# congkaishen/MotionPlanning

Hardware: AMD Instinct MI355X
Metric: MPPI rollouts/s (K×H dyn+cost steps/s) at K=8192,H=50; 1/2/4/8 GPU (higher is better)
Workload: dtype f64

## Files before the change

motionplanning_amd/csrc/mppi.hip:

```cpp
#include "mppi_device.hpp"
#include "runtime.hpp"

#include <hip/hip_ext.h>

#include <algorithm>
#include <cstdlib>
#include <type_traits>
#include <vector>

using namespace mpk;

namespace {

constexpr int NT = 256;
constexpr int RPB = NT / 2;
#ifndef MPPI_PRIO
#define MPPI_PRIO 3
#endif
constexpr size_t kMaxLds = 146 * 1024;
constexpr size_t kCoLds = 70 * 1024;

__device__ __forceinline__ double block_reduce_min(double v, double* sh) {
  for (int o = 32; o >= 1; o >>= 1) v = nanmin(v, __shfl_xor(v, o));
  const int w = threadIdx.x >> 6;
// ... 39 lines not shown
  int* rc_out;
  int* fc_out;
  int nb;
  int pstride;
  int lds_unom, lds_obs, lds_grid;
  int lds_cq;
  int lds_ctrl, lds_part;
  unsigned long long* stamps;
  int inline_noise;
  double* fin;
  int fin_stride;
  const int* live;
};

#ifndef MPPI_NT_CTRL
#define MPPI_NT_CTRL 0
#endif

struct FinRec {
  int u, unom, x0, goal, obs, grid, ran, stride;
  __host__ __device__ FinRec(int H, int n_obs, int gbytes) {
    u = 0;
    unom = 2 * H;
    x0 = 4 * H;
    goal = x0 + 7;
    obs = goal + 2;
    grid = obs + 3 * n_obs;
    ran = grid + (gbytes + 7) / 8;
    stride = (ran + 2) & ~1;
  }
};

#define MP_STAMP(i)                                                                  \
  do {                                                                               \
    if (A.stamps && threadIdx.x == 0) {                                              \
      A.stamps[blockIdx.x * 32 + (i)] = __builtin_amdgcn_s_memrealtime();            \
      if ((i) == 0) {                                                                \
        unsigned xcc;                                                                \
        asm volatile("s_getreg_b32 %0, hwreg(HW_REG_XCC_ID)" : "=s"(xcc));           \
        A.stamps[blockIdx.x * 32 + 30] = xcc;                                        \
      }                                                                              \
    }                                                                                \
  } while (0)
#define MP_STAMP_WAVE()                                                              \
  do {                                                                               \
    if (A.stamps && (threadIdx.x & 63) == 0) {                                       \
      unsigned hwid;                                                                 \
      asm volatile("s_getreg_b32 %0, hwreg(HW_REG_HW_ID)" : "=s"(hwid));             \
      A.stamps[blockIdx.x * 32 + 8 + (threadIdx.x >> 6)] = __builtin_amdgcn_s_memrealtime(); \
      A.stamps[blockIdx.x * 32 + 20 + (threadIdx.x >> 6)] = hwid;                    \
    }                                                                                \
  } while (0)

__global__ __launch_bounds__(256) void noise_prep_kernel(MppiDev P, int S, const double* ext, double* zh) {
  const long long i = (long long)blockIdx.x * blockDim.x + threadIdx.x;
  const long long n = (long long)S * P.H * P.K;
  if (i >= n) return;
  const int k = (int)(i % P.K);
  const long long t = i / P.K;
  const int h = (int)(t % P.H), s = (int)(t / P.H);
  double z[2];
  if (P.noise_mode == 0) {
    const double2 e = *reinterpret_cast<const double2*>(ext + (((size_t)s * P.K + k) * P.H + h) * 2);
    z[0] = e.x;
    z[1] = e.y;
  } else {
    philox_normal2(P, (unsigned)s, (unsigned)k, (unsigned)h, z);
  }
  reinterpret_cast<double2*>(zh)[i] = make_double2(z[0], z[1]);
}

template <class T>
__device__ __forceinline__ void st_ag(T* p, T v) {
  __hip_atomic_store(p, v, __ATOMIC_RELAXED, __HIP_MEMORY_SCOPE_AGENT);
}
template <class T>
__device__ __forceinline__ T ld_ag(const T* p) {
  return __hip_atomic_load(const_cast<T*>(p), __ATOMIC_RELAXED, __HIP_MEMORY_SCOPE_AGENT);
}
#ifndef MPPI_COHERENT_PARTS
#define MPPI_COHERENT_PARTS 0
#endif

template <int BT, int LPR, bool INL>
__global__ __launch_bounds__(BT) void mppi_plan_kernel(MppiDev P, PlanArgs A) {
  constexpr int NT = BT, RPB = BT / LPR, NQ = BT / 128;
  constexpr bool WPART = LPR == 2;
  __shared__ double sh_red[NT / 64];
  __shared__ double sh_e[RPB];
  __shared__ double sh_q[WPART ? NT / 64 : NQ][128];
  __shared__ int sh_last, sh_m, sh_bstar, sh_fc;
  __shared__ double sh_eta;
  __shared__ double atab[kTabDoubles];
  extern __shared__ double dyn[];
  const int H = P.H, H2 = 2 * H, K = P.K;
  const int s = blockIdx.x / A.nb, b = blockIdx.x % A.nb;
  const int tid = threadIdx.x, pair = LPR == 2 ? tid >> 1 : tid, side = LPR == 2 ? tid & 1 : 0;
  const int k = b * RPB + pair;
  const bool active = k < K;
  const int kk = active ? k : K - 1;
  if (A.live && A.live[s] == 0) {
    if (A.fin && b == 0 && tid == 0) A.fin[(size_t)s * A.fin_stride + FinRec(H, P.n_obs, P.gnx * P.gny).ran] = 0.0;
    return;
  }
  MP_STAMP(0);
  __builtin_amdgcn_s_setprio(3);

  const double* X0 = A.X0 + 7 * s;
  const double* goal = A.goal + 2 * s;
  const double* noise = A.noise ? A.noise + (size_t)K * H2 * s : nullptr;
  double* unom = dyn + A.lds_unom;
  double* obs = A.obs ? dyn + A.lds_obs : nullptr;
  double* ush = A.lds_ctrl >= 0 ? dyn + A.lds_ctrl : nullptr;
  const int ustr = H2 + 1;
  const unsigned char* grid = nullptr;
  {
    const double* gu = A.unom + (size_t)H2 * s;
    rollout_tab_fill(atab, P, tid, NT);
    for (int i = tid; i < H2; i += NT) unom[i] = gu[i];
    if (P.ctrl_cost)
      for (int i = tid; i < H; i += NT) ctrl_cost_row(P, gu[2 * i], gu[2 * i + 1], dyn + A.lds_cq + 2 * i);
    if (A.obs) {
      const double* go = A.obs + (size_t)3 * P.n_obs * s;
      for (int i = tid; i < 3 * P.n_obs; i += NT) obs[i] = go[i];
    }
    if (A.grid) {
      const int gb = P.gnx * P.gny;
      const unsigned char* gg = A.grid + (size_t)gb * s;
      if (A.lds_grid >= 0) {
        unsigned char* lg = reinterpret_cast<unsigned char*>(dyn + A.lds_grid);
        for (int i = tid; i < gb; i += NT) lg[i] = gg[i];
        grid = lg;
      } else {
        grid = gg;
      }
    }
    __syncthreads();
  }
  double* ctrl_g = A.ctrl_all ? A.ctrl_all + ((size_t)s * H * K + kk) * 2 + side : nullptr;

#if MPPI_PRIO == 3
  __shared__ int sh_simd[NT / 64];
  __shared__ volatile int sh_prog[NT / 64];
  const int wv = __builtin_amdgcn_readfirstlane(tid >> 6);
  int sib = -1;
  {
    unsigned hw;
    asm volatile("s_getreg_b32 %0, hwreg(HW_REG_HW_ID)" : "=s"(hw));
    if ((tid & 63) == 0) {
      sh_simd[wv] = (int)((hw >> 4) & 3u);
      sh_prog[wv] = 0;
    }
    __syncthreads();
    const int me = sh_simd[wv];
    for (int w = 0; w < NT / 64; w++)
      if (w != wv && sh_simd[w] == me) sib = w;
    sib = __builtin_amdgcn_readfirstlane(sib);
  }
  int sib_j = 0;
#endif
  int feas;
  double c;
  {
    const double2* zrow = noise ? reinterpret_cast<const double2*>(noise) + kk : nullptr;
    double2 zc = zrow ? zrow[0] : make_double2(0.0, 0.0), zn = zc;
    auto ctrl = [&](int j, double* u) {
      double2 zj;
      if (INL && LPR == 1) {
        double zz[2];
        philox_normal2(P, (unsigned)s, (unsigned)kk, (unsigned)j, zz);
        zj = make_double2(zz[0], zz[1]);
      } else if (INL) {
        if ((j & 1) == 0) {
          double zz[2];
          philox_normal2(P, (unsigned)s, (unsigned)kk, (unsigned)(j + side), zz);
          const double o0 = pair_swap(zz[0]), o1 = pair_swap(zz[1]);
          zj = side ? make_double2(o0, o1) : make_double2(zz[0], zz[1]);
          zn = side ? make_double2(zz[0], zz[1]) : make_double2(o0, o1);
        } else {
          zj = zn;
        }
      } else {
        zj = zc;
        if (j + 1 < H) zc = zrow[(size_t)(j + 1) * K];
      }
      const double z[2] = {zj.x, zj.y};
      sample_ctrl(P, z, unom + 2 * j, u);
#if MPPI_PRIO == 0
      if ((4 * j) % H < 4 && j > 0) {
        const int q = (4 * j) / H;
        if (q == 1) __builtin_amdgcn_s_setprio(2);
        else if (q == 2) __builtin_amdgcn_s_setprio(1);
        else if (q == 3) __builtin_amdgcn_s_setprio(0);
      }
#elif MPPI_PRIO == 3
      if (sib >= 0) {
        const int o = __builtin_amdgcn_readfirstlane(sib_j);
        if (j > o) __builtin_amdgcn_s_setprio(0);
        else if (j < o) __builtin_amdgcn_s_setprio(2);
        else __builtin_amdgcn_s_setprio(1);
        sh_prog[wv] = j;
        sib_j = sh_prog[sib];
      } else if ((4 * j) % H < 4 && j > 0) {
        const int q = (4 * j) / H;
        if (q == 1) __builtin_amdgcn_s_setprio(2);
        else if (q == 2) __builtin_amdgcn_s_setprio(1);
        else if (q == 3) __builtin_amdgcn_s_setprio(0);
      }
#else
      if (j > 0) {
        const int t1 = MPPI_PRIO == 1 ? H / 2 : H - 12, t2 = MPPI_PRIO == 1 ? 3 * H / 4 : H - 6,
                  t3 = MPPI_PRIO == 1 ? 7 * H / 8 : H - 3;
        if (j == t1) __builtin_amdgcn_s_setprio(2);
        else if (j == t2) __builtin_amdgcn_s_setprio(1);
        else if (j == t3) __builtin_amdgcn_s_setprio(0);
      }
#endif
    };
    auto store = [&](int j, const double* u) {
      if (LPR == 2) {
        if (ush) ush[pair * ustr + 2 * j + side] = u[side];
        if (ctrl_g) {
#if MPPI_NT_CTRL
          __builtin_nontemporal_store(u[side], ctrl_g + (size_t)j * K * 2);
#else
          ctrl_g[(size_t)j * K * 2] = u[side];
#endif
        }
      } else {
        if (ush) {
          ush[pair * ustr + 2 * j] = u[0];
          ush[pair * ustr + 2 * j + 1] = u[1];
        }
        if (ctrl_g) *reinterpret_cast<double2*>(ctrl_g + (size_t)j * K * 2) = make_double2(u[0], u[1]);
      }
    };
    const TrajOut traj{A.coll_traj ? A.coll_traj + (size_t)s * (H + 1) * 7 * K + kk : nullptr, 7LL * K, (long long)K};
    c = rollout_pair<LPR>(P, X0, goal, obs, grid, unom, side, ctrl, store, traj, &feas, atab, dyn + A.lds_cq);
  }
  MP_STAMP(1);
  MP_STAMP_WAVE();
  if (active && side == 0) {
    st_ag(A.cost_all + (size_t)s * K + k, c);
    st_ag(A.feas_all + (size_t)s * K + k, (unsigned char)feas);
    if (c != c) atomicOr(A.flags, 1);
  }
  const int wid = tid >> 6, lane = tid & 63;
  const bool wp = WPART && H2 <= 128;
  const int nr = wp ? max(0, min(32, K - b * RPB - 32 * wid)) : 0;
  constexpr bool PREF = BT == 512;
  double v0[32], v1[32];
  if (PREF && wp && !ush) {
    asm volatile("s_waitcnt vmcnt(0)" ::: "memory");
    const double* cb = A.ctrl_all + (((size_t)s * H + (lane >> 1)) * K + (size_t)b * RPB + 32 * wid) * 2 + (lane & 1);
    const size_t up = (size_t)64 * K;
#pragma unroll
    for (int r = 0; r < 32; r++) v0[r] = (r < nr && lane < H2) ? cb[2 * r] : 0.0;
    if (H2 > 64) {
#pragma unroll
      for (int r = 0; r < 32; r++) v1[r] = (r < nr && lane + 64 < H2) ? cb[up + 2 * r] : 0.0;
    }
  }
  const double cm = active ? c : __builtin_inf();
  const double rho_b = block_reduce_min(cm, sh_red);
  const double e = active ? mpj_exp(P.nil * (c - rho_b)) : 0.0;
  if (side == 0) sh_e[pair] = e;
  const double eta_b = block_reduce_sum(side == 0 ? e : 0.0, sh_red);
  const double fc_b = block_reduce_sum((side == 0 && active && feas) ? 1.0 : 0.0, sh_red);
  __syncthreads();
  double* part = A.part + ((size_t)s * A.nb + b) * A.pstride;
  if (wp) {
    const double* ew = sh_e + 32 * wid;
    double a0 = 0.0, a1 = 0.0;
    if (ush) {
      const double* uw = ush + (size_t)(32 * wid) * ustr + lane;
      for (int r = 0; r < nr; r++) {
        const double er = ew[r];
        if (lane < H2) a0 = a0 + er * uw[r * ustr];
        if (lane + 64 < H2) a1 = a1 + er * uw[r * ustr + 64];
      }
    } else if (PREF) {
#pragma unroll
      for (int r = 0; r < 32; r++) {
        if (r < nr) {
          const double er = ew[r];
          a0 = a0 + er * v0[r];
          if (H2 > 64) a1 = a1 + er * v1[r];
        }
      }
    } else {
      const double* cb = A.ctrl_all + (((size_t)s * H + (lane >> 1)) * K + (size_t)b * RPB + 32 * wid) * 2 + (lane & 1);
      const size_t up = (size_t)64 * K;
      for (int r = 0; r < nr; r++) {
        const double er = ew[r];
        if (lane < H2) a0 = a0 + er * cb[2 * r];
        if (lane + 64 < H2) a1 = a1 + er * cb[up + 2 * r];
      }
    }
    sh_q[wid][lane] = a0;
    sh_q[wid][lane + 64] = a1;
    __syncthreads();
    if (tid < H2) {
      double v = sh_q[0][tid];
#pragma unroll
      for (int w = 1; w < NT / 64; w++) v = v + sh_q[w][tid];
      st_ag(part + 4 + tid, v);
    }
  } else {
    const int t = tid % 128, q = tid / 128;
    const int r0 = q * (RPB / NQ), r1 = r0 + RPB / NQ;
    for (int t0 = 0; t0 < H2; t0 += 128) {
      const int tt = t0 + t;
      double acc = 0.0;
      if (tt < H2) {
        if (ush) {
          for (int r = r0; r < r1; r++) acc = acc + sh_e[r] * ush[r * ustr + tt];
        } else {
          const double* cb = A.ctrl_all + (((size_t)s * H + (tt >> 1)) * K + (size_t)b * RPB) * 2 + (tt & 1);
          const int rmax = min(r1, K - b * RPB);
#pragma unroll 16
          for (int r = r0; r < rmax; r++) acc = acc + sh_e[r] * cb[(size_t)r * 2];
// ... 328 lines not shown
      for (int k = 0; k < 7; k++) states[7 * vv + k] = x[k];
      if (last >= max_steps) live[vv] = 0;
    }
  }
}

__host__ __device__ inline int shard_rec(int H) { return 2 * H + 7 * (H + 1) + 4; }

__global__ __launch_bounds__(256) void shard_pack_kernel(int S, int H, const double* U, const double* traj,
                                                         const double* cost, const int* feas, const int* rc,
                                                         const int* fc, double* out) {
  const int D = shard_rec(H), nu = 2 * H, nt = 7 * (H + 1);
  const long long i = (long long)blockIdx.x * 256 + threadIdx.x;
  if (i >= (long long)S * D) return;
  const int s = (int)(i / D), j = (int)(i % D);
  double v;
  if (j < nu) v = U[(size_t)s * nu + j];
  else if (j < nu + nt) v = traj[(size_t)s * nt + (j - nu)];
  else {
    const int q = j - nu - nt;
    v = q == 0 ? cost[s] : q == 1 ? (double)feas[s] : q == 2 ? (double)rc[s] : (double)fc[s];
  }
  out[i] = v;
}

static void inv2(const double* A, double* Ai) {
  const double a = A[0], b = A[1], c = A[2], d = A[3];
  if (b == 0.0 && c == 0.0) {
    Ai[0] = 1.0 / a; Ai[1] = 0.0; Ai[2] = 0.0; Ai[3] = 1.0 / d;
    return;
  }
  const bool swap = __builtin_fabs(c) > __builtin_fabs(a);
  const double p11 = swap ? c : a, p12 = swap ? d : b, q11 = swap ? a : c, q12 = swap ? b : d;
  const double l = q11 / p11, u22 = q12 - l * p12;
  const double iu11 = 1.0 / p11, iu22 = 1.0 / u22, iu12 = -(p12 * iu11) * iu22;
  const double m11 = iu11 - iu12 * l, m12 = iu12, m21 = -iu22 * l, m22 = iu22;
  if (swap) { Ai[0] = m12; Ai[1] = m11; Ai[2] = m22; Ai[3] = m21; }
  else { Ai[0] = m11; Ai[1] = m12; Ai[2] = m21; Ai[3] = m22; }
}

static int make_dev_params(mp_ctx* ctx, const mp_mppi_params* p, int K, MppiDev* D) {
  MP_CHECK(ctx, p != nullptr, "params is NULL");
  MP_CHECK(ctx, K >= 1, "SamplingNumber K (%d) must be >= 1", K);
  MP_CHECK(ctx, p->H >= 1 && p->H <= 4096, "horizon N (%d) must be in [1, 4096]", p->H);
  MP_CHECK(ctx, p->n_obs >= 0, "n_obs (%d) must be >= 0", p->n_obs);
  MP_CHECK(ctx, p->dt > 0.0, "dt (%g) must be > 0", p->dt);
  MP_CHECK(ctx, p->grid_nx >= 0 && p->grid_ny >= 0, "grid dims must be >= 0");
  MP_CHECK(ctx, p->noise_mode == MP_NOISE_EXTERNAL || p->noise_mode == MP_NOISE_PHILOX, "bad noise_mode %d",
           p->noise_mode);
  MP_CHECK(ctx, p->calls_in_flight >= 0 && p->calls_in_flight <= 64, "calls_in_flight (%d) must be in [0, 64]",
           p->calls_in_flight);
  D->in_flight = p->calls_in_flight > 1 ? p->calls_in_flight : 1;
  D->K = K;
  D->H = p->H;
  D->FC = p->feasibility_count;
  D->n_obs = p->n_obs;
  D->dt = p->dt;
  D->lambda = p->lambda;
  D->nil = (-1.0) / p->lambda;
  const double* S = p->sigma;
  MP_CHECK(ctx, S[0] > 0.0, "Σ must be positive definite");
  const double l11 = __builtin_sqrt(S[0]);
  const double l21 = S[2] / l11;
  const double r22 = S[3] - l21 * l21;
  MP_CHECK(ctx, r22 > 0.0, "Σ must be positive definite");
  D->L[0] = l11; D->L[1] = 0.0; D->L[2] = l21; D->L[3] = __builtin_sqrt(r22);
  inv2(S, D->Si);
  for (int i = 0; i < 7; i++) { D->XL[i] = p->XL[i]; D->XU[i] = p->XU[i]; }
  for (int i = 0; i < 2; i++) { D->CL[i] = p->CL[i]; D->CU[i] = p->CU[i]; }
  D->slack = p->slack_penalty;
  D->obs_pen = p->obs_penalty;
  D->gnx = p->grid_nx;
  D->gny = p->grid_ny;
  D->gx0 = p->grid_x0; D->gy0 = p->grid_y0; D->gdx = p->grid_dx; D->gdy = p->grid_dy;
  D->noise_mode = p->noise_mode;
  D->ctrl_cost = p->ctrl_cost;
  D->seed = p->seed;
  D->offset = p->offset;
  D->scene_base = p->scene_base;
  return MP_OK;
}

using PlanFn = void (*)(MppiDev, PlanArgs);
static PlanFn plan_kernel_for(int BT, int LPR, bool inl) {
#define MP_PLAN_CASE(bt, lpr) \
  if (BT == bt && LPR == lpr) return inl ? mppi_plan_kernel<bt, lpr, true> : mppi_plan_kernel<bt, lpr, false>;
  MP_PLAN_CASE(128, 1)
  MP_PLAN_CASE(128, 2)
  MP_PLAN_CASE(256, 1)
  MP_PLAN_CASE(256, 2)
  MP_PLAN_CASE(512, 1)
  MP_PLAN_CASE(512, 2)
#undef MP_PLAN_CASE
  return nullptr;
}

static int plan_launch(mp_ctx* ctx, const MppiDev& D, int S, const double* X0, const double* goal,
                       const double* U_nom, const double* obstacles, const uint8_t* grid, const double* noise,
                       double* U_out, double* traj_out, double* cost_out, int32_t* feasible_out,
                       int32_t* rc_out, int32_t* fc_out, double* coll_traj, double* coll_ctrl,
                       double* coll_cost, uint8_t* coll_feas, int final_stream, const int* live = nullptr) {
  const int K = D.K, H = D.H;
  const char* lpr_s = getenv("MPGPU_LPR");
  const int lpr_env = lpr_s ? atoi(lpr_s) : 0;
  const int LPR = lpr_env == 1 || lpr_env == 2 ? lpr_env : ((size_t)S * K * D.in_flight >= 131072 ? 1 : 2);
  const int BT = LPR == 1 ? ((size_t)S * ((K + 511) / 512) >= 256 ? 512 : 256)
                          : ((size_t)S * ((K + 255) / 256) >= 256 ? 512 : 256);
  const int RPBh = BT / LPR;
  const int nb = (K + RPBh - 1) / RPBh;
  const int pstride = 4 + 2 * H;
  PlanArgs A;
  A.live = live;
  A.X0 = X0; A.goal = goal; A.unom = U_nom; A.obs = D.n_obs > 0 ? obstacles : nullptr;
  A.grid = D.gnx > 0 ? grid : nullptr;
  A.inline_noise = D.noise_mode == MP_NOISE_PHILOX;
  A.noise = nullptr;
  if (!A.inline_noise) {
    double* zh = (double*)mp_ws(ctx, WS_NOISE, sizeof(double) * (size_t)S * K * H * 2);
    if (!zh) return MP_ERR_NOMEM;
    const long long n = (long long)S * K * H;
    hipLaunchKernelGGL(noise_prep_kernel, dim3((unsigned)((n + 255) / 256)), dim3(256), 0, ctx->stream, D, S, noise,
                       zh);
    MP_HIP(ctx, hipGetLastError());
    A.noise = zh;
  }
  A.cost_all = coll_cost ? coll_cost : (double*)mp_ws(ctx, WS_MPPI_COST, sizeof(double) * (size_t)S * K);
  A.feas_all = coll_feas ? coll_feas : (unsigned char*)mp_ws(ctx, WS_MPPI_FEAS, (size_t)S * K);
  A.part = (double*)mp_ws(ctx, WS_MPPI_PART, sizeof(double) * (size_t)S * nb * pstride);
  if (!A.cost_all || !A.feas_all || !A.part) return MP_ERR_NOMEM;
  A.coll_traj = coll_traj;
  int st = mp_ticket_reserve(ctx, S);
  if (st) return st;
  A.tickets = ctx->tickets;
  A.flags = ctx->flags;
  A.U_out = U_out; A.traj_out = traj_out; A.cost_out = cost_out; A.feas_out = feasible_out;
  A.rc_out = rc_out; A.fc_out = fc_out;
  A.nb = nb;
  A.pstride = pstride;
  int off = 2 * H + nb;
  A.lds_unom = off;
  off += 2 * H;
  A.lds_cq = off;
  off += 2 * H;
  A.lds_obs = off;
  off += 3 * D.n_obs;
  const size_t gbytes = (size_t)D.gnx * D.gny;
  A.lds_grid = -1;
  if (D.gnx > 0 && (size_t)off * 8 + gbytes <= 48 * 1024) {
    A.lds_grid = off;
    off += (int)((gbytes + 7) / 8);
  }
  const int ctrl_words = RPBh * (2 * H + 1), part_words = nb * pstride;
  A.lds_ctrl = A.lds_part = -1;
  const bool many = (size_t)S * nb > 256;
  const size_t budget = many ? kCoLds : kMaxLds;
  if ((size_t)(off + (ctrl_words > part_words ? ctrl_words : part_words)) * 8 <= budget) {
    A.lds_ctrl = A.lds_part = off;
    off += ctrl_words > part_words ? ctrl_words : part_words;
  } else if ((size_t)(off + part_words) * 8 <= budget) {
    A.lds_part = off;
    off += part_words;
  }
  A.ctrl_all = coll_ctrl;
  if (A.lds_ctrl < 0 && !A.ctrl_all) {
    A.ctrl_all = (double*)mp_ws(ctx, WS_IO14, sizeof(double) * (size_t)S * K * 2 * H);
    if (!A.ctrl_all) return MP_ERR_NOMEM;
  }
  const size_t shmem = sizeof(double) * (size_t)off;
  MP_CHECK(ctx, shmem <= kMaxLds, "K/H/obstacles too large for one scene (dynamic LDS %zu B)", shmem);
  if (!ctx->mppi_lds_attr) {
    MP_HIP(ctx, hipSetDevice(ctx->device));
    for (int bt : {128, 256, 512})
      for (int lpr : {1, 2})
        for (bool inl : {false, true})
          MP_HIP(ctx, hipFuncSetAttribute((const void*)plan_kernel_for(bt, lpr, inl),
                                          hipFuncAttributeMaxDynamicSharedMemorySize, (int)kMaxLds));
    ctx->mppi_lds_attr = true;
  }
  A.fin = nullptr;
  A.fin_stride = 0;
  int par = 0;
  if (final_stream) {
    int st2 = mp_side_init(ctx);
    if (st2) return st2;
    par = ctx->fin_par;
    ctx->fin_par = (par + 1) % MP_FIN_RING;
    const FinRec R(H, D.n_obs, D.gnx * D.gny);
    A.fin_stride = R.stride;
    for (int q = 0; q < MP_FIN_RING; q++)
      if (!mp_ws(ctx, WS_FIN0 + q, sizeof(double) * (size_t)S * R.stride)) return MP_ERR_NOMEM;
    A.fin = (double*)mp_ws(ctx, WS_FIN0 + par, sizeof(double) * (size_t)S * R.stride);
    MP_HIP(ctx, hipEventSynchronize(ctx->ev_fin[par]));
  }
  A.stamps = nullptr;
  static const bool stamps_on = getenv("MPGPU_STAMPS") != nullptr;
  if (stamps_on) {
    A.stamps = (unsigned long long*)mp_ws(ctx, WS_HA2, sizeof(unsigned long long) * 32 * S * nb);
    MP_HIP(ctx, hipMemsetAsync(A.stamps, 0, sizeof(unsigned long long) * 32 * S * nb, ctx->stream));
  }
  hipEvent_t t_start, t_stop;
  mp_time_pair(ctx, &t_start, &t_stop);
  const dim3 grd(S * nb);
  {
    MppiDev Dl = D;
    void* args[] = {(void*)&Dl, (void*)&A};
    MP_HIP(ctx, hipExtLaunchKernel((const void*)plan_kernel_for(BT, LPR, A.inline_noise != 0), grd, dim3(BT), args,
                                   shmem, ctx->stream, t_start, t_stop, 0));
  }
  MP_HIP(ctx, hipGetLastError());
  if (final_stream) {
    const FinRec R(H, D.n_obs, D.gnx * D.gny);
    const int grid_lds = (size_t)R.stride * 8 <= 64 * 1024;
    const size_t fsh = sizeof(double) * (size_t)(grid_lds ? R.stride : R.grid);
    MP_CHECK(ctx, fsh <= kMaxLds, "final rollout snapshot too large for LDS (%zu B)", fsh);
    if (!ctx->fin_lds_attr) {
      MP_HIP(ctx, hipSetDevice(ctx->device));
      MP_HIP(ctx, hipFuncSetAttribute((const void*)final_rollout_kernel, hipFuncAttributeMaxDynamicSharedMemorySize,
                                      (int)kMaxLds));
      ctx->fin_lds_attr = true;
    }
    hipEvent_t plan_done = t_stop;
    if (!plan_done) {
      plan_done = ctx->ev_plan[par];
      MP_HIP(ctx, hipEventRecord(plan_done, ctx->stream));
    }
    MP_HIP(ctx, hipStreamWaitEvent(ctx->side, plan_done, 0));
    hipLaunchKernelGGL(final_rollout_kernel, dim3(S), dim3(64), fsh, ctx->side, D, A.fin, A.fin_stride, grid_lds,
                       traj_out, cost_out, feasible_out, ctx->flags);
    MP_HIP(ctx, hipGetLastError());
    MP_HIP(ctx, hipEventRecord(ctx->ev_fin[par], ctx->side));
  }
  if (stamps_on) {
    std::vector<unsigned long long> h(32 * S * nb);
    MP_HIP(ctx, hipMemcpyAsync(h.data(), A.stamps, h.size() * 8, hipMemcpyDeviceToHost, ctx->stream));
    MP_HIP(ctx, hipStreamSynchronize(ctx->stream));
    unsigned long long t0 = ~0ull, end = 0;
    double d01 = 0, d12 = 0, d23 = 0;
    int last = -1;
    for (int b = 0; b < S * nb; b++) {
      const unsigned long long* q = &h[32 * b];
      t0 = q[0] < t0 ? q[0] : t0;
      d01 += (q[1] - q[0]) / 100.0; d12 += (q[2] - q[1]) / 100.0; d23 += (q[3] - q[2]) / 100.0;
      if (q[5]) last = b;
      end = q[5] > end ? q[5] : end;
      end = q[3] > end ? q[3] : end;
    }
    fprintf(stderr, "[stamps us] blocks=%d mean rollout %.2f partial %.2f ticket %.2f", S * nb, d01 / (S * nb),
            d12 / (S * nb), d23 / (S * nb));
    {
      std::vector<double> st, en;
      for (int b = 0; b < S * nb; b++) {
        st.push_back((h[32 * b] - t0) / 100.0);
        en.push_back((h[32 * b + 1] - t0) / 100.0);
      }
      std::sort(st.begin(), st.end());
      std::sort(en.begin(), en.end());
      const int n = S * nb;
      fprintf(stderr, " | start p0/50/90/100 %.1f %.1f %.1f %.1f | p1-end p0/50/90/100 %.1f %.1f %.1f %.1f", st[0],
              st[n / 2], st[n * 9 / 10], st[n - 1], en[0], en[n / 2], en[n * 9 / 10], en[n - 1]);
      std::vector<double> we;
      int hist[9] = {0};
      for (int b = 0; b < n; b++) {
        int cnt[4] = {0, 0, 0, 0}, mx = 0;
        for (int w = 0; w < 8; w++) {
          const unsigned long long tw = h[32 * b + 8 + w];
          if (!tw) continue;
          we.push_back((tw - t0) / 100.0);
          const int simd = (int)((h[32 * b + 20 + w] >> 4) & 3);
          mx = std::max(mx, ++cnt[simd]);
        }
        hist[mx]++;
      }
      std::sort(we.begin(), we.end());
      const int m = (int)we.size();
      fprintf(stderr, " | wave-end p0/50/90/100 %.1f %.1f %.1f %.1f | blocks by max waves/SIMD 1:%d 2:%d 3:%d 4:%d",
              we[0], we[m / 2], we[m * 9 / 10], we[m - 1], hist[1], hist[2], hist[3], hist[4]);
    }
    {
      double sum[16] = {0}, mx[16] = {0};
      int cnt[16] = {0}, nbk[16] = {0};
      for (int b = 0; b < S * nb; b++) {
        const int x = (int)(h[32 * b + 30] & 15);
        nbk[x]++;
        for (int w = 0; w < 8; w++) {
          const unsigned long long tw = h[32 * b + 8 + w];
          if (!tw) continue;
          const double v = (tw - t0) / 100.0;
          sum[x] += v; cnt[x]++; mx[x] = std::max(mx[x], v);
        }
// ... 404 lines not shown
```

motionplanning_amd/csrc/mppi_device.hpp:

```cpp
#pragma once
#include <hip/hip_runtime.h>

#include "../../include/mp_jlmath.h"

namespace mpk {

struct MppiDev {
  int K, H, FC, n_obs;
  double dt, lambda, nil;
  double L[4];
  double Si[4];
  double XL[7], XU[7], CL[2], CU[2];
  double slack, obs_pen;
  int gnx, gny;
  double gx0, gy0, gdx, gdy;
  int noise_mode, ctrl_cost;
  unsigned long long seed, offset;
  int scene_base;
  int in_flight;
};

__device__ __forceinline__ double pair_swap(double v) {
  const int lo = __builtin_amdgcn_mov_dpp(__double2loint(v), 0xB1, 0xF, 0xF, false);
  const int hi = __builtin_amdgcn_mov_dpp(__double2hiint(v), 0xB1, 0xF, 0xF, false);
// ... 29 lines not shown
  return k;
}
__device__ __forceinline__ void dyn_pair_sc(const double* x, double sr, double ax, double* d, int side,
                                            const double* atab, double sp, double cp, const PairK& pk) {
  const double g = 9.81, mu = 0.8, KFZX = 186.22;
  const double B = -10.4 / mu, C = 1.3, E = 0.1556;
  const double v = x[2], r = x[3], ux = x[5], sa = x[6];
  const double t = (ax - r * v) * KFZX;
  const double FZ = 2 * (pk.kfz * g + t * pk.tsg);
  const double alpha = TY_ATAN(mpj_div_g(v + pk.lr * r, ux + 0.01), atab) - (side ? 0.0 : sa);
  const double X1 = B * alpha;
  const double FY = mu * FZ * 1.0 * TY_SIN(C * TY_ATAN(X1 - E * (X1 - TY_ATAN(X1, atab)), atab));
  const double FYo = pair_swap(FY);
  const double uxc = MPJ_SEL(ux <= 0, 0.0, ux);
  d[0] = uxc * cp - v * sp;
  d[1] = uxc * sp + v * cp;
  const double q = mpj_div_gn(FY * pk.cown + FYo * pk.cother, pk.div, pk.rdiv, 1);
  const double qo = pair_swap(q);
  d[2] = (side ? qo : q) - r * uxc;
  d[3] = side ? q : qo;
  d[4] = r;
  d[5] = ax;
  d[6] = sr;
}
__device__ __forceinline__ void dyn_pair(const double* x, double sr, double ax, double* d, int side, const double* atab) {
  double sp, cp;
  TY_SINCOS(x[4], &sp, &cp);
  dyn_pair_sc(x, sr, ax, d, side, atab, sp, cp, pair_k(side));
}

struct LaneK {
  double rM, rI;
};
__device__ __forceinline__ LaneK lane_k() {
  LaneK k;
  k.rM = mpj_rcp_nr(2020.0);
  k.rI = mpj_rcp_nr(4095.0);
  return k;
}
__device__ __forceinline__ void dyn_lane(const double* x, double sr, double ax, double* d, const double* atab,
                                         const LaneK& lk) {
  const double la = 1.56, lb = 1.64, M = 2020.0, Izz = 4095.0, g = 9.81, mu = 0.8;
  const double KFZF = 1018.28 / 2, KFZR = 963.34 / 2, KFZX = 186.22;
  const double B = -10.4 / mu, C = 1.3, E = 0.1556;
  const double v = x[2], r = x[3], psi = x[4], ux = x[5], sa = x[6];
  const double t = (ax - r * v) * KFZX;
  const double FZf = 2 * (KFZF * g + -t), FZr = 2 * (KFZR * g + t);
  double qf, qr;
  mpj_div2_g(v + la * r, v + (-lb) * r, ux + 0.01, &qf, &qr);
  const double af = TY_ATAN(qf, atab) - sa;
  const double ar = TY_ATAN(qr, atab) - 0.0;
  const double Xf = B * af, Xr = B * ar;
  const double FY1 = mu * FZf * 1.0 * TY_SIN(C * TY_ATAN(Xf - E * (Xf - TY_ATAN(Xf, atab)), atab));
  const double FY2 = mu * FZr * 1.0 * TY_SIN(C * TY_ATAN(Xr - E * (Xr - TY_ATAN(Xr, atab)), atab));
  const double uxc = MPJ_SEL(ux <= 0, 0.0, ux);
  double sp, cp;
  TY_SINCOS(psi, &sp, &cp);
  d[0] = uxc * cp - v * sp;
  d[1] = uxc * sp + v * cp;
  d[2] = mpj_div_gn(FY1 + FY2, M, lk.rM, 1) - r * uxc;
  d[3] = mpj_div_gn(FY1 * la - FY2 * lb, Izz, lk.rI, 1);
  d[4] = r;
  d[5] = ax;
  d[6] = sr;
}

__device__ __forceinline__ double run_cost(const double* x, double sr, double ax) {
  const double y = x[1], v = x[2], r = x[3], sa = x[6];
  return v * v * 1 + 1 * (r * r) + 5 * (ax * ax) + 3 * (sr * sr) + 2 * (sa * sa) + 10 * (y * y);
}

struct GridK {
  double rx, ry;
  int ok;
};
template <int LPR = 2>
__device__ __forceinline__ GridK grid_k(const MppiDev& P, int side) {
  GridK g;
  g.rx = mpj_rcp_nr(LPR == 2 && side ? P.gdy : P.gdx);
  g.ry = mpj_rcp_nr(P.gdy);
  g.ok = P.gnx > 0 && !mpj_div_out(P.gdx) && !mpj_div_out(P.gdy);
  return g;
}
template <int LPR = 2>
__device__ __forceinline__ double obstacle_cost(const MppiDev& P, const double* x, const double* obs,
                                                const unsigned char* grid, int* ok, int side, const GridK& gk) {
  double c = 0.0;
  for (int o = 0; o < P.n_obs; o++) {
    const double dx = x[0] - obs[3 * o], dy = x[1] - obs[3 * o + 1], R = obs[3 * o + 2];
    const int hit = dx * dx + dy * dy <= R * R;
    *ok &= !hit;
    c = (hit ? c + P.obs_pen : c);
  }
  if (P.gnx > 0) {
    double fx, fy;
    if (LPR == 2) {
      const double f = mpj_div_gn(side ? x[1] - P.gy0 : x[0] - P.gx0, side ? P.gdy : P.gdx, gk.rx, gk.ok);
      const double fo = pair_swap(f);
      fx = side ? fo : f;
      fy = side ? f : fo;
    } else {
      fx = mpj_div_gn(x[0] - P.gx0, P.gdx, gk.rx, gk.ok);
      fy = mpj_div_gn(x[1] - P.gy0, P.gdy, gk.ry, gk.ok);
    }
    const int inb = fx >= 0.0 && fy >= 0.0 && fx < (double)P.gnx && fy < (double)P.gny;
    const int ix = inb ? (int)fx : 0, iy = inb ? (int)fy : 0;
    const int hit = inb && grid[iy * P.gnx + ix];
    *ok &= !hit;
    c = (hit ? c + P.obs_pen : c);
  }
  return c;
}

constexpr int kTabBnd = 4 * MPJ_ATAN_ROWS, kTabDoubles = kTabBnd + 14;
__device__ __forceinline__ void rollout_tab_fill(double* tab, const MppiDev& P, unsigned tid, unsigned step) {
  mpj_atan_rows_fill(tab, tid, step);
  if (tid == 0) {
#pragma unroll
    for (int i = 0; i < 7; i++) {
      tab[kTabBnd + 2 * i] = P.XL[i];
      tab[kTabBnd + 2 * i + 1] = P.XU[i];
    }
  }
}

__device__ __forceinline__ double bound_cost(const MppiDev& P, const double* bnd, const double* x, int* ok) {
  asm volatile("" : "+v"(bnd));
  int viol = 0;
#pragma unroll
  for (int i = 0; i < 7; i++) viol |= (x[i] < bnd[2 * i]) | (x[i] > bnd[2 * i + 1]);
  *ok &= !viol;
  double c = 0.0;
  if (__any(viol)) {
#pragma unroll
    for (int i = 0; i < 7; i++) {
      const double xl = bnd[2 * i], xu = bnd[2 * i + 1];
      const int lo = x[i] < xl, hi = x[i] > xu;
      const double vl = c + P.slack * __builtin_fabs(x[i] - xl);
      c = lo ? vl : c;
      const double vh = c + P.slack * __builtin_fabs(x[i] - xu);
      c = hi ? vh : c;
    }
  }
  return c;
}

__device__ __forceinline__ void philox4x32(unsigned c0, unsigned c1, unsigned c2, unsigned c3, unsigned k0,
                                           unsigned k1, unsigned* o) {
  asm volatile("" : "+s"(k0), "+s"(k1));
#pragma unroll
  for (int i = 0; i < 10; i++) {
    const unsigned long long p0 = (unsigned long long)0xD2511F53u * c0;
    const unsigned long long p1 = (unsigned long long)0xCD9E8D57u * c2;
    const unsigned hi0 = (unsigned)(p0 >> 32), lo0 = (unsigned)p0;
    const unsigned hi1 = (unsigned)(p1 >> 32), lo1 = (unsigned)p1;
    const unsigned n0 = hi1 ^ c1 ^ k0, n2 = hi0 ^ c3 ^ k1;
    c0 = n0;
    c1 = lo1;
    c2 = n2;
    c3 = lo0;
    k0 += 0x9E3779B9u;
    k1 += 0xBB67AE85u;
  }
  o[0] = c0;
  o[1] = c1;
  o[2] = c2;
  o[3] = c3;
}

__device__ __forceinline__ void philox_normal2(const MppiDev& P, unsigned scene, unsigned k, unsigned h,
                                               double* z) {
  unsigned o[4];
  philox4x32(k, h, scene + (unsigned)P.scene_base, (unsigned)P.offset, (unsigned)P.seed,
             (unsigned)(P.seed >> 32) ^ (unsigned)(P.offset >> 32), o);
  const unsigned long long b1 = ((unsigned long long)(o[0] >> 5) << 26) | (unsigned long long)(o[1] >> 6);
  const unsigned long long b2 = ((unsigned long long)(o[2] >> 5) << 26) | (unsigned long long)(o[3] >> 6);
  const double u1 = ((double)b1 + 0.5) * 1.1102230246251565e-16;
  const double u2 = ((double)b2 + 0.5) * 1.1102230246251565e-16;
  const double rr = mpj_sqrt(-2.0 * mpj_log_bl(u1));
  double sn, cs;
  mpj_sincos_bl(MPJ_TWO_PI * u2, &sn, &cs);
  z[0] = rr * cs;
  z[1] = rr * sn;
}

__device__ __forceinline__ void sample_ctrl(const MppiDev& P, const double* z, const double* un, double* u) {
  const double n0 = P.L[0] * z[0];
  const double n1 = P.L[3] * z[1] + P.L[2] * z[0];
  const double v0 = n0 + un[0], v1 = n1 + un[1];
  const double c0 = __builtin_fmin(__builtin_fmax(v0, P.CL[0]), P.CU[0]);
  const double c1 = __builtin_fmin(__builtin_fmax(v1, P.CL[1]), P.CU[1]);
  u[0] = v0 != v0 ? v0 : c0;
  u[1] = v1 != v1 ? v1 : c1;
}

__device__ __forceinline__ void draw_ctrl(const MppiDev& P, const double* noise_s, const double* unom_s,
                                          unsigned scene, int k, int h, double* u) {
  double z[2];
  if (P.noise_mode == 0) {
    const double2 zz = *reinterpret_cast<const double2*>(noise_s + ((size_t)k * P.H + h) * 2);
    z[0] = zz.x;
    z[1] = zz.y;
  } else {
    philox_normal2(P, scene, (unsigned)k, (unsigned)h, z);
  }
  sample_ctrl(P, z, unom_s + 2 * h, u);
}

struct TrajOut {
  double* p;
  long long rs, cs;
};

#ifndef MPPI_NT_STATE
#define MPPI_NT_STATE 1
#endif
__device__ __forceinline__ void st_state(double* a, double v) {
  if (MPPI_NT_STATE) __builtin_nontemporal_store(v, a);
  else *a = v;
}
template <int LPR = 2>
__device__ __forceinline__ void store_state(const TrajOut& T, int j, const double* x, int side) {
  double* q = T.p + (long long)j * T.rs;
  if (LPR == 1) {
#pragma unroll
    for (int i = 0; i < 7; i++) st_state(q + (long long)i * T.cs, x[i]);
    return;
  }
#pragma unroll
  for (int i = 0; i < 4; i++) {
    const double v = MPJ_SEL(side, x[4 + i < 7 ? 4 + i : 6], x[i]);
    if (!side || i < 3) st_state(q + (long long)(side ? 4 + i : i) * T.cs, v);
  }
}

__device__ __forceinline__ void ctrl_cost_row(const MppiDev& P, double un0, double un1, double* t) {
  const double a0 = P.lambda * un0, a1 = P.lambda * un1;
  t[0] = __builtin_fma(P.Si[0], a0, P.Si[2] * a1);
  t[1] = __builtin_fma(P.Si[1], a0, P.Si[3] * a1);
}

template <int LPR = 2, class CtrlFn, class StoreFn>
__device__ __forceinline__ double rollout_pair(const MppiDev& P, const double* X0, const double* goal,
                                               const double* obs, const unsigned char* grid,
                                               const double* unom, int side, CtrlFn ctrl, StoreFn store,
                                               const TrajOut& traj, int* feas, const double* atab,
                                               const double* cq = nullptr) {
  double x[7];
#pragma unroll
  for (int i = 0; i < 7; i++) x[i] = X0[i];
  const PairK pk = pair_k(side);
  const LaneK lk = lane_k();
  const GridK gk = grid_k<LPR>(P, side);
  if (traj.p) store_state<LPR>(traj, 0, x, side);
  double sum = 0.0;
  int ok_all = 1;
  for (int j = 0; j < P.H; j++) {
    double u[2];
    ctrl(j, u);
    store(j, u);
    int okc = 1, okb = 1;
    double cc = 0.0, cb = 0.0;
    if (j > 0) {
      cc = obstacle_cost<LPR>(P, x, obs, grid, &okc, side, gk);
      cb = bound_cost(P, atab + kTabBnd, x, &okb);
    }
    const double pc = run_cost(x, u[0], u[1]);
    double k1[7], k2[7], x2[7];
    if (LPR == 2) {
      const double psi2 = x[4] + x[3] * P.dt;
      double sn, cs;
      TY_SINCOS(side ? psi2 : x[4], &sn, &cs);
      const double so = pair_swap(sn), co = pair_swap(cs);
      dyn_pair_sc(x, u[0], u[1], k1, side, atab, side ? so : sn, side ? co : cs, pk);
#pragma unroll
      for (int i = 0; i < 7; i++) x2[i] = x[i] + k1[i] * P.dt;
      dyn_pair_sc(x2, u[0], u[1], k2, side, atab, side ? sn : so, side ? cs : co, pk);
    } else {
      dyn_lane(x, u[0], u[1], k1, atab, lk);
#pragma unroll
      for (int i = 0; i < 7; i++) x2[i] = x[i] + k1[i] * P.dt;
      dyn_lane(x2, u[0], u[1], k2, atab, lk);
    }
#pragma unroll
    for (int i = 0; i < 7; i++) x[i] = x[i] + P.dt * (k1[i] + k2[i]) / 2;
    double cj = pc + cb + cc;
    if (P.ctrl_cost) {
      const double un0 = unom[2 * j], un1 = unom[2 * j + 1];
      double t[2];
      if (cq) {
        t[0] = cq[2 * j];
        t[1] = cq[2 * j + 1];
      } else {
        ctrl_cost_row(P, un0, un1, t);
      }
      const double d0 = u[0] - un0, d1 = u[1] - un1;
      cj = cj + __builtin_fma(t[1], d1, t[0] * d0);
    }
    sum = sum + cj;
    ok_all &= okc & okb;
    if (traj.p) store_state<LPR>(traj, j + 1, x, side);
  }
  {
    int okc = 1, okb = 1;
    const double pc = run_cost(x, 0.0, 0.0);
    const double cc = obstacle_cost<LPR>(P, x, obs, grid, &okc, side, gk);
    const double cb = bound_cost(P, atab + kTabBnd, x, &okb);
    sum = sum + (pc + cb + cc);
    ok_all &= okc & okb;
  }
  const double tx = x[0] - goal[0], ty = x[1] - goal[1];
  const double term = tx * tx + ty * ty;
  const double dx0 = X0[0] - goal[0], dy0 = X0[1] - goal[1];
  *feas = ok_all;
  return sum + term / (dx0 * dx0 + dy0 * dy0) * 10000.0;
}

__device__ __forceinline__ double nanmin(double a, double b) { return (a != a || a < b) ? a : b; }

}
```

Measured before the change: 17.66 billion.

## Add lean specialized plan kernel with uniform-base stores and compile-time branches

Adds a LEAN template instance of the MPPI plan kernel, picked automatically when the configuration matches: inline noise, one rollout per lane, grid in LDS, no circle obstacles, control cost on, trajectory and control collection on. It removes runtime branches (obstacle loop, ctrl_cost and traj pointer checks) at compile time. It uses SGPR base plus VGPR 32-bit offset addressing for control and state stores, with explicit LDS/global address spaces, to cut VGPR pressure and 64-bit address arithmetic. It also drops the LDS control staging buffer in that path. The costs are another kernel instance, the K < 2^27 offset limit, and a slightly different priority-step schedule.

```diff
diff --git a/motionplanning_amd/csrc/mppi.hip b/motionplanning_amd/csrc/mppi.hip
--- a/motionplanning_amd/csrc/mppi.hip
+++ b/motionplanning_amd/csrc/mppi.hip
@@ -145,8 +145,9 @@
 #define MPPI_COHERENT_PARTS 0
 #endif
 
-template <int BT, int LPR, bool INL>
+template <int BT, int LPR, bool INL, bool LEAN = false>
 __global__ __launch_bounds__(BT) void mppi_plan_kernel(MppiDev P, PlanArgs A) {
+  static_assert(!LEAN || (INL && LPR == 1), "lean instance: device noise, one rollout per lane");
   constexpr int NT = BT, RPB = BT / LPR, NQ = BT / 128;
   constexpr bool WPART = LPR == 2;
   __shared__ double sh_red[NT / 64];
@@ -173,24 +174,24 @@
   const double* goal = A.goal + 2 * s;
   const double* noise = A.noise ? A.noise + (size_t)K * H2 * s : nullptr;
   double* unom = dyn + A.lds_unom;
-  double* obs = A.obs ? dyn + A.lds_obs : nullptr;
-  double* ush = A.lds_ctrl >= 0 ? dyn + A.lds_ctrl : nullptr;
+  double* obs = !LEAN && A.obs ? dyn + A.lds_obs : nullptr;
+  double* ush = !LEAN && A.lds_ctrl >= 0 ? dyn + A.lds_ctrl : nullptr;
   const int ustr = H2 + 1;
   const unsigned char* grid = nullptr;
   {
     const double* gu = A.unom + (size_t)H2 * s;
     rollout_tab_fill(atab, P, tid, NT);
     for (int i = tid; i < H2; i += NT) unom[i] = gu[i];
-    if (P.ctrl_cost)
+    if (LEAN || P.ctrl_cost)
       for (int i = tid; i < H; i += NT) ctrl_cost_row(P, gu[2 * i], gu[2 * i + 1], dyn + A.lds_cq + 2 * i);
-    if (A.obs) {
+    if (!LEAN && A.obs) {
       const double* go = A.obs + (size_t)3 * P.n_obs * s;
       for (int i = tid; i < 3 * P.n_obs; i += NT) obs[i] = go[i];
     }
-    if (A.grid) {
+    if (LEAN || A.grid) {
       const int gb = P.gnx * P.gny;
       const unsigned char* gg = A.grid + (size_t)gb * s;
-      if (A.lds_grid >= 0) {
+      if (LEAN || A.lds_grid >= 0) {
         unsigned char* lg = reinterpret_cast<unsigned char*>(dyn + A.lds_grid);
         for (int i = tid; i < gb; i += NT) lg[i] = gg[i];
         grid = lg;
@@ -201,6 +202,10 @@
     __syncthreads();
   }
   double* ctrl_g = A.ctrl_all ? A.ctrl_all + ((size_t)s * H * K + kk) * 2 + side : nullptr;
+  unsigned long long ctrl_u = LEAN ? reinterpret_cast<unsigned long long>(A.ctrl_all + (size_t)s * H * K * 2) : 0;
+  unsigned ctrl_off = (unsigned)kk * 16u;
+  const unsigned ctrl_row = (unsigned)K * 16u;
+  const int pq1 = (H + 3) >> 2, pq2 = (2 * H + 3) >> 2, pq3 = (3 * H + 3) >> 2;
 
 #if MPPI_PRIO == 3
   __shared__ int sh_simd[NT / 64];
@@ -262,8 +267,18 @@
         if (j > o) __builtin_amdgcn_s_setprio(0);
         else if (j < o) __builtin_amdgcn_s_setprio(2);
         else __builtin_amdgcn_s_setprio(1);
-        sh_prog[wv] = j;
-        sib_j = sh_prog[sib];
+        if (LEAN) {
+          typedef __attribute__((address_space(3))) volatile int* lds_vip;
+          ((lds_vip)sh_prog)[wv] = j;
+          sib_j = ((lds_vip)sh_prog)[sib];
+        } else {
+          sh_prog[wv] = j;
+          sib_j = sh_prog[sib];
+        }
+      } else if (LEAN) {
+        if (j == pq3) __builtin_amdgcn_s_setprio(0);
+        else if (j == pq2) __builtin_amdgcn_s_setprio(1);
+        else if (j == pq1) __builtin_amdgcn_s_setprio(2);
       } else if ((4 * j) % H < 4 && j > 0) {
         const int q = (4 * j) / H;
         if (q == 1) __builtin_amdgcn_s_setprio(2);
@@ -281,7 +296,11 @@
 #endif
     };
     auto store = [&](int j, const double* u) {
-      if (LPR == 2) {
+      if (LEAN) {
+        typedef double d2v __attribute__((ext_vector_type(2)));
+        *reinterpret_cast<__attribute__((address_space(1))) d2v*>(uni_addr(ctrl_u, ctrl_off)) = d2v{u[0], u[1]};
+        ctrl_u += ctrl_row;
+      } else if (LPR == 2) {
         if (ush) ush[pair * ustr + 2 * j + side] = u[side];
         if (ctrl_g) {
 #if MPPI_NT_CTRL
@@ -298,8 +317,14 @@
         if (ctrl_g) *reinterpret_cast<double2*>(ctrl_g + (size_t)j * K * 2) = make_double2(u[0], u[1]);
       }
     };
-    const TrajOut traj{A.coll_traj ? A.coll_traj + (size_t)s * (H + 1) * 7 * K + kk : nullptr, 7LL * K, (long long)K};
-    c = rollout_pair<LPR>(P, X0, goal, obs, grid, unom, side, ctrl, store, traj, &feas, atab, dyn + A.lds_cq);
+    if constexpr (LEAN) {
+      const TrajUni traj{reinterpret_cast<unsigned long long>(A.coll_traj + (size_t)s * (H + 1) * 7 * K), (unsigned)kk * 8u,
+                         (unsigned)K * 8u};
+      c = rollout_pair<LPR, true>(P, X0, goal, obs, grid, unom, side, ctrl, store, traj, &feas, atab, dyn + A.lds_cq);
+    } else {
+      const TrajOut traj{A.coll_traj ? A.coll_traj + (size_t)s * (H + 1) * 7 * K + kk : nullptr, 7LL * K, (long long)K};
+      c = rollout_pair<LPR>(P, X0, goal, obs, grid, unom, side, ctrl, store, traj, &feas, atab, dyn + A.lds_cq);
+    }
   }
   MP_STAMP(1);
   MP_STAMP_WAVE();
@@ -794,7 +819,12 @@
 }
 
 using PlanFn = void (*)(MppiDev, PlanArgs);
-static PlanFn plan_kernel_for(int BT, int LPR, bool inl) {
+static PlanFn plan_kernel_for(int BT, int LPR, bool inl, bool lean = false) {
+  if (lean) {
+    if (BT == 256 && LPR == 1 && inl) return mppi_plan_kernel<256, 1, true, true>;
+    if (BT == 512 && LPR == 1 && inl) return mppi_plan_kernel<512, 1, true, true>;
+    return nullptr;
+  }
 #define MP_PLAN_CASE(bt, lpr) \
   if (BT == bt && LPR == lpr) return inl ? mppi_plan_kernel<bt, lpr, true> : mppi_plan_kernel<bt, lpr, false>;
   MP_PLAN_CASE(128, 1)
@@ -866,7 +896,16 @@
   A.lds_ctrl = A.lds_part = -1;
   const bool many = (size_t)S * nb > 256;
   const size_t budget = many ? kCoLds : kMaxLds;
-  if ((size_t)(off + (ctrl_words > part_words ? ctrl_words : part_words)) * 8 <= budget) {
+  const char* lean_s = getenv("MPGPU_PLAN_LEAN");
+  const bool lean = !(lean_s && lean_s[0] == '0' && !lean_s[1]) && LPR == 1 && (BT == 256 || BT == 512) && A.inline_noise &&
+                    D.n_obs == 0 && A.grid && A.lds_grid >= 0 && D.ctrl_cost && coll_traj && coll_ctrl &&
+                    K < (1 << 27);
+  if (lean) {
+    if ((size_t)(off + part_words) * 8 <= budget) {
+      A.lds_part = off;
+      off += part_words;
+    }
+  } else if ((size_t)(off + (ctrl_words > part_words ? ctrl_words : part_words)) * 8 <= budget) {
     A.lds_ctrl = A.lds_part = off;
     off += ctrl_words > part_words ? ctrl_words : part_words;
   } else if ((size_t)(off + part_words) * 8 <= budget) {
@@ -887,6 +926,9 @@
         for (bool inl : {false, true})
           MP_HIP(ctx, hipFuncSetAttribute((const void*)plan_kernel_for(bt, lpr, inl),
                                           hipFuncAttributeMaxDynamicSharedMemorySize, (int)kMaxLds));
+    for (int bt : {256, 512})
+      MP_HIP(ctx, hipFuncSetAttribute((const void*)plan_kernel_for(bt, 1, true, true),
+                                      hipFuncAttributeMaxDynamicSharedMemorySize, (int)kMaxLds));
     ctx->mppi_lds_attr = true;
   }
   A.fin = nullptr;
@@ -916,7 +958,7 @@
   {
     MppiDev Dl = D;
     void* args[] = {(void*)&Dl, (void*)&A};
-    MP_HIP(ctx, hipExtLaunchKernel((const void*)plan_kernel_for(BT, LPR, A.inline_noise != 0), grd, dim3(BT), args,
+    MP_HIP(ctx, hipExtLaunchKernel((const void*)plan_kernel_for(BT, LPR, A.inline_noise != 0, lean), grd, dim3(BT), args,
                                    shmem, ctx->stream, t_start, t_stop, 0));
   }
   MP_HIP(ctx, hipGetLastError());
diff --git a/motionplanning_amd/csrc/mppi_device.hpp b/motionplanning_amd/csrc/mppi_device.hpp
--- a/motionplanning_amd/csrc/mppi_device.hpp
+++ b/motionplanning_amd/csrc/mppi_device.hpp
@@ -135,17 +135,17 @@
   g.ok = P.gnx > 0 && !mpj_div_out(P.gdx) && !mpj_div_out(P.gdy);
   return g;
 }
-template <int LPR = 2>
+template <int LPR = 2, bool LEAN = false>
 __device__ __forceinline__ double obstacle_cost(const MppiDev& P, const double* x, const double* obs,
                                                 const unsigned char* grid, int* ok, int side, const GridK& gk) {
   double c = 0.0;
-  for (int o = 0; o < P.n_obs; o++) {
+  for (int o = 0; !LEAN && o < P.n_obs; o++) {
     const double dx = x[0] - obs[3 * o], dy = x[1] - obs[3 * o + 1], R = obs[3 * o + 2];
     const int hit = dx * dx + dy * dy <= R * R;
     *ok &= !hit;
     c = (hit ? c + P.obs_pen : c);
   }
-  if (P.gnx > 0) {
+  if (LEAN || P.gnx > 0) {
     double fx, fy;
     if (LPR == 2) {
       const double f = mpj_div_gn(side ? x[1] - P.gy0 : x[0] - P.gx0, side ? P.gdy : P.gdx, gk.rx, gk.ok);
@@ -177,7 +177,8 @@
   }
 }
 
-__device__ __forceinline__ double bound_cost(const MppiDev& P, const double* bnd, const double* x, int* ok) {
+template <class BndP>
+__device__ __forceinline__ double bound_cost(const MppiDev& P, BndP bnd, const double* x, int* ok) {
   asm volatile("" : "+v"(bnd));
   int viol = 0;
 #pragma unroll
@@ -196,6 +197,11 @@
     }
   }
   return c;
+}
+
+typedef __attribute__((address_space(3))) const double* mp_lds_cdp;
+__device__ __forceinline__ double bound_cost_lds(const MppiDev& P, const double* bnd, const double* x, int* ok) {
+  return bound_cost(P, (mp_lds_cdp)bnd, x, ok);
 }
 
 __device__ __forceinline__ void philox4x32(unsigned c0, unsigned c1, unsigned c2, unsigned c3, unsigned k0,
@@ -264,6 +270,19 @@
   double* p;
   long long rs, cs;
 };
+__device__ __forceinline__ bool traj_on(const TrajOut& T) { return T.p != nullptr; }
+struct TrajUni {
+  unsigned long long base;
+  unsigned off;
+  unsigned cs;
+};
+__device__ __forceinline__ bool traj_on(const TrajUni&) { return true; }
+typedef __attribute__((address_space(1))) char mp_gchar;
+__device__ __forceinline__ mp_gchar* uni_addr(unsigned long long& base, unsigned& off) {
+  asm volatile("" : "+s"(base));
+  asm volatile("" : "+v"(off));
+  return reinterpret_cast<mp_gchar*>(base) + (size_t)off;
+}
 
 #ifndef MPPI_NT_STATE
 #define MPPI_NT_STATE 1
@@ -273,6 +292,17 @@
   else *a = v;
 }
 template <int LPR = 2>
+__device__ __forceinline__ void store_state(TrajUni& T, int, const double* x, int) {
+  static_assert(LPR == 1, "uniform-base stores: one rollout per lane");
+#pragma unroll
+  for (int i = 0; i < 7; i++) {
+    auto* q = reinterpret_cast<__attribute__((address_space(1))) double*>(uni_addr(T.base, T.off));
+    if (MPPI_NT_STATE) __builtin_nontemporal_store(x[i], q);
+    else *q = x[i];
+    T.base += T.cs;
+  }
+}
+template <int LPR = 2>
 __device__ __forceinline__ void store_state(const TrajOut& T, int j, const double* x, int side) {
   double* q = T.p + (long long)j * T.rs;
   if (LPR == 1) {
@@ -293,19 +323,20 @@
   t[1] = __builtin_fma(P.Si[1], a0, P.Si[3] * a1);
 }
 
-template <int LPR = 2, class CtrlFn, class StoreFn>
+template <int LPR = 2, bool LEAN = false, class CtrlFn, class StoreFn, class TrajT>
 __device__ __forceinline__ double rollout_pair(const MppiDev& P, const double* X0, const double* goal,
                                                const double* obs, const unsigned char* grid,
                                                const double* unom, int side, CtrlFn ctrl, StoreFn store,
-                                               const TrajOut& traj, int* feas, const double* atab,
+                                               const TrajT& traj_, int* feas, const double* atab,
                                                const double* cq = nullptr) {
+  TrajT traj = traj_;
   double x[7];
 #pragma unroll
   for (int i = 0; i < 7; i++) x[i] = X0[i];
   const PairK pk = pair_k(side);
   const LaneK lk = lane_k();
   const GridK gk = grid_k<LPR>(P, side);
-  if (traj.p) store_state<LPR>(traj, 0, x, side);
+  if (traj_on(traj)) store_state<LPR>(traj, 0, x, side);
   double sum = 0.0;
   int ok_all = 1;
   for (int j = 0; j < P.H; j++) {
@@ -315,8 +346,8 @@
     int okc = 1, okb = 1;
     double cc = 0.0, cb = 0.0;
     if (j > 0) {
-      cc = obstacle_cost<LPR>(P, x, obs, grid, &okc, side, gk);
-      cb = bound_cost(P, atab + kTabBnd, x, &okb);
+      cc = obstacle_cost<LPR, LEAN>(P, x, obs, grid, &okc, side, gk);
+      cb = LEAN ? bound_cost_lds(P, atab + kTabBnd, x, &okb) : bound_cost(P, atab + kTabBnd, x, &okb);
     }
     const double pc = run_cost(x, u[0], u[1]);
     double k1[7], k2[7], x2[7];
@@ -338,10 +369,10 @@
 #pragma unroll
     for (int i = 0; i < 7; i++) x[i] = x[i] + P.dt * (k1[i] + k2[i]) / 2;
     double cj = pc + cb + cc;
-    if (P.ctrl_cost) {
+    if (LEAN || P.ctrl_cost) {
       const double un0 = unom[2 * j], un1 = unom[2 * j + 1];
       double t[2];
-      if (cq) {
+      if (LEAN || cq) {
         t[0] = cq[2 * j];
         t[1] = cq[2 * j + 1];
       } else {
@@ -352,13 +383,13 @@
     }
     sum = sum + cj;
     ok_all &= okc & okb;
-    if (traj.p) store_state<LPR>(traj, j + 1, x, side);
+    if (traj_on(traj)) store_state<LPR>(traj, j + 1, x, side);
   }
   {
     int okc = 1, okb = 1;
     const double pc = run_cost(x, 0.0, 0.0);
-    const double cc = obstacle_cost<LPR>(P, x, obs, grid, &okc, side, gk);
-    const double cb = bound_cost(P, atab + kTabBnd, x, &okb);
+    const double cc = obstacle_cost<LPR, LEAN>(P, x, obs, grid, &okc, side, gk);
+    const double cb = LEAN ? bound_cost_lds(P, atab + kTabBnd, x, &okb) : bound_cost(P, atab + kTabBnd, x, &okb);
     sum = sum + (pc + cb + cc);
     ok_all &= okc & okb;
   }
```

Measured after the change: 18.63 billion, median of 6. 1.05x the previous value.
